# indianajohn/akaze-rust

Hardware: AMD Instinct MI355X
Metric: Mpix/s through extract_features (4 oct x 4 sub) (higher is better)
Workload: dtype f32

## Files before the change

akaze-rust_amd/csrc/akz_ctx.hpp:

```cpp
#pragma once
#include <algorithm>
#include <cmath>
#include <cstdlib>
#include <cstddef>
#include <cstring>
#include <atomic>
#include <condition_variable>
#include <functional>
#include <map>
#include <memory>
#include <mutex>
#include <thread>
#include <sched.h>
#include <time.h>
#include <type_traits>

#include "akz_internal.hpp"
#include "akz_select.hpp"
#include "akz_pool.hpp"
#include "akz_gates.hpp"

#define AKZ_LOCAL __attribute__((visibility("hidden")))

namespace akz {
// ... 51 lines not shown
    DevBuf kp_in, kp_out;
    DevBuf match_a, match_b, match_rec, match_out;
    DevBuf match_state;
    uint32_t match_epoch = 0;
    DevBuf ransac_dev, ransac_pin;
    DevBuf mm_q8, mm_t8, mm_pop, mm_tab;
    DevBuf mm_cols;
    void* tab_ring = nullptr;
    size_t tab_ring_bytes = 0;
    uint64_t tab_ring_next = 0;
    hipEvent_t tab_ring_ev[4] = {nullptr, nullptr, nullptr, nullptr};
    struct MatchSide {
        DevBuf q8, t8, pop, tab, cols, rec;
        void* ring = nullptr;
        size_t ring_bytes = 0;
        uint64_t ring_next = 0;
        hipEvent_t ring_ev[4] = {nullptr, nullptr, nullptr, nullptr};
    } ms1;
    int match_mode = 2;
    uint32_t dbg_pair_chunks = 0, dbg_set_chunks = 0;
    int dbg_device_libm = -1;
    int libm_last = 0;
    int dbg_host_sort = -1;
    DevBuf cosi;
    DevBuf pin[10];
    std::vector<std::pair<size_t, void*>> slab_pool;
    std::mutex slab_m;
    static constexpr int kSlots = 3;
    DevBuf cand_slot[kSlots], count_slot[kSlots];
    std::atomic<bool> slot_busy[kSlots] = {{false}, {false}, {false}};
    std::atomic<uint32_t> cand_cap_hint{1u << 15};
    std::atomic<int> live_results{0};
    bool dead = false;
    std::atomic<uint32_t> last_total_cands{0};
    std::atomic<uint64_t> last_cand_shape{0};
    hipStream_t aux = nullptr;
    std::mutex aux_m;
    hipStream_t coarse = nullptr;
    hipStream_t pre = nullptr;
    hipEvent_t pre_done = nullptr;
    hipStream_t copy = nullptr;
    DevBuf stage[kSlots];
    hipEvent_t staged[kSlots] = {nullptr, nullptr, nullptr};
    std::vector<akz_ctx*> lanes;
    unsigned next_lane = 0;
    bool is_lane = false;
    bool eager_finish = true;
    std::shared_ptr<Finisher> fin;
    hipEvent_t lane_in = nullptr;
    uint64_t stream_min_px = gates::kStreamPx;
    int prep_mode = 2;
    int det_mode = 2;
    int fed_mode = 2;
    int sched[11] = {0, 1, 0, 0, 0, 0, 0, 0, 0, 0, 0};
    uint64_t big_px = gates::kBigPxAsync;
    uint64_t big_px_sync = gates::kBigPxSync, big_px_async = gates::kBigPxAsync;
    uint64_t lane_px = gates::kLanePx;
    static constexpr uint64_t kLaunchMarchPx = gates::kMarchPx;
    uint64_t launch_min_px = kLaunchMarchPx;
    bool placed = false;
    int pre_mode = 0;
    int place_replaced = 0;
    int place_collisions = 0;
    int place_retries = 0;
    int lane_collisions = 0;
    hipEvent_t probe_ev[2] = {nullptr, nullptr};
    int profiling = 0;
    akz_profile prof{};
    struct Span { int stage; hipEvent_t a, b; int row; };
    std::vector<Span> spans;
    std::vector<akz_kernel_row> rows;
    std::vector<hipEvent_t> ev_pool;
    std::mutex ev_m;
    static constexpr int kFedRing = 4;
    hipEvent_t fed_ev[kFedRing] = {nullptr, nullptr, nullptr, nullptr};
    hipEvent_t pre_ev[kFedRing] = {nullptr, nullptr, nullptr, nullptr};
    std::atomic<uint64_t> begin_seq{0};
    std::shared_ptr<std::atomic<int>> in_hand = std::make_shared<std::atomic<int>>(0);
    std::unique_ptr<WorkerPool> workers;
    unsigned host_threads = 0;
    WorkerPool& pool() {
        if (!workers) workers.reset(new WorkerPool(std::min(host_threads ? host_threads : host_cpu_share(), 16u) - 1));
        return *workers;
    }
    hipStream_t fetch[2] = {nullptr, nullptr};
    DevBuf fetch_stage;
    hipEvent_t fetch_chunk[4] = {nullptr, nullptr, nullptr, nullptr};
    DevBuf fetch_tmp[3], fetch_out[2][4];
    hipEvent_t fetch_start = nullptr, fetch_join = nullptr, fetch_ready[2] = {nullptr, nullptr}, fetch_free[2] = {nullptr, nullptr};
    static constexpr int kJpegSlots = 16;
    DevBuf jpeg_pin[kJpegSlots];
    hipEvent_t jpeg_up[kJpegSlots] = {};
    DevBuf jpeg_coef, jpeg_plane, jpeg_frames;
    std::mutex jpeg_m;
};
constexpr int kStageIngest = 10;

struct StageTimer {
    akz_ctx* c;
    int stage;
    hipEvent_t a = nullptr, b = nullptr;
    static hipEvent_t get(akz_ctx* c) {
        {
            std::lock_guard<std::mutex> lk(c->ev_m);
            if (!c->ev_pool.empty()) {
                hipEvent_t e = c->ev_pool.back();
                c->ev_pool.pop_back();
// ... 169 lines not shown
```

akaze-rust_amd/csrc/akz_extract.cpp:

```cpp
#include "akz_ctx.hpp"

struct akz_result {
    akz_ctx* ctx = nullptr;
    akz_config cfg;
    uint32_t w = 0, h = 0, n = 0, flags = 0;
    uint64_t big_px = 0;
    std::vector<LevelPlan> plan;
    void* slab = nullptr;
    size_t slab_bytes = 0;
    float* planes[kMaxLevels][10];
    double* d_k = nullptr;
    std::vector<double> k_host;
    std::vector<std::vector<akz_keypoint>> kps;
    std::vector<uint8_t> rows64;
    uint8_t* d_desc64 = nullptr;
    size_t desc_block_bytes = 0;
    std::vector<uint64_t> desc_off;
    std::vector<uint64_t> n_extrema;
};

static size_t align_up(size_t v, size_t a) { return (v + a - 1) / a * a; }

static int slab_acquire(akz_ctx* c, size_t bytes, void** p, size_t* got) {
    bytes = align_up(std::max<size_t>(bytes, 256), 256);
// ... 498 lines not shown
    std::vector<char> prepared(L + 1, 0);
    const uint64_t level_min_px = gates::kLevelMarchPx;
    auto takes_level_march = [&](size_t l) {
        return !plan[l].tau.empty() && c->fed_mode == 2 && launch::level_march_supported(plan[l].w, plan[l].h) &&
               (c->prep_mode == 3 || (c->prep_mode == 2 && (uint64_t)plan[l].w * plan[l].h * n >= level_min_px));
    };
    auto takes_stream_prep = [&](size_t l) {
        const bool half_l = plan[l].octave > plan[l - 1].octave;
        return c->prep_mode != 0 && launch::prep_stream_supported(plan[l].w, plan[l].h) &&
               (c->prep_mode == 1 || (c->prep_mode >= 2 && !half_l && (uint64_t)plan[l].w * plan[l].h * n >= c->stream_min_px));
    };
    auto run_levels = [&](size_t lo, size_t hi) -> int {
    for (size_t i = lo; i < hi; ++i) {
        const LevelPlan& lv = plan[i];
        const LevelPlan& pv = plan[i - 1];
        if (i >= 2) interleave_detector(i - 1);

        if (i == res_first) {
            std::vector<launch::ResidentLevel> rl;
            std::vector<std::vector<float>> ht(L);
            uint64_t px_steps = 0;
            for (size_t l = i; l < L; ++l) {
                for (double t : plan[l].tau) ht[l].push_back(0.5f * (float)t);
                rl.push_back(launch::ResidentLevel{P(l, AKZ_LT), P(l, AKZ_LSMOOTH), P(l, AKZ_LFLOW), keep_all ? P(l, AKZ_LSTEP) : nullptr,
                                                   plan[l].w, plan[l].h, plan[l].octave > plan[l - 1].octave,
                                                   (uint32_t)plan[l].tau.size(), ht[l].data(), plan[l].octave});
                px_steps += (uint64_t)plan[l].w * plan[l].h * n * plan[l].tau.size();
            }
            StageTimer st(c, AKZ_ST_FED);
            st.kernel(AKZ_KR_OCTAVE_RESIDENT, (uint32_t)rl.size(), plan[i].w, plan[i].h, n, 1, 0, px_steps);
            launch::octave_resident(ls, P(i - 1, AKZ_LT), pv.w, pv.h, n, rl.data(), (uint32_t)rl.size(), g1.data(), r->d_k);
            if (c->profiling) {
                c->prof.fed_launches += 1;
                c->prof.fed_px_steps += px_steps;
            }
            AKZ_HIP_TRY(hipGetLastError());
            break;
        }
        float* A = P(i, AKZ_LT);
        const bool on_coarse = i >= fork_level;
        if (on_coarse) AKZ_TRY(ensure(c, c->scratch_coarse, plane_bytes(plan[fork_level].w, plan[fork_level].h, n)));
        float* B = (float*)(on_coarse ? c->scratch_coarse.p : c->scratch[5].p);
        const uint32_t n_tau = (uint32_t)lv.tau.size();
        const bool half = lv.octave > pv.octave;
        const float* fed_in = P(i - 1, AKZ_LT);
        float* half_buf = nullptr;
        if (half) {
            const uint32_t launches = fed_num_launches(c, n_tau, lv.w, lv.h, n);
            half_buf = launches == 0 ? A : (fed_dst(launches, 1, A, B) == A ? B : A);
            fed_in = half_buf;
        }
        const bool fuse_level = takes_level_march(i);
        if (fuse_level) {
            const uint32_t n1 = std::min<uint32_t>(n_tau, 4u), rem = n_tau - n1;
            const uint32_t rest = rem ? fed_num_launches(c, rem, lv.w, lv.h, n) : 0;
            float* d1 = fed_dst(rest + 1, 1, A, B);
            const float* level_in = P(i - 1, AKZ_LT);
            const bool fold_half = half && launch::level_march_half_supported(lv.w, lv.h, pv.w, pv.h, n1);
            if (half && !fold_half) {
                StageTimer st(c, AKZ_ST_PREP);
                float* hb = d1 == A ? B : A;
                launch::half_size(ls, P(i - 1, AKZ_LT), hb, pv.w, pv.h, n);
                level_in = hb;
            }
            float ht[4];
            for (uint32_t j = 0; j < n1; ++j) ht[j] = 0.5f * (float)lv.tau[j];
            {
                StageTimer st(c, AKZ_ST_FED);
                st.kernel(AKZ_KR_LEVEL_MARCH, n1 | (fold_half ? 16u : 0u) | ((rem == 0 && keep_all) ? 32u : 0u), lv.w, lv.h, n, 1,
                          (uint64_t)lv.w * lv.h * n, (uint64_t)lv.w * lv.h * n * n1);
                launch::level_march(ls, level_in, P(i, AKZ_LSMOOTH), P(i, AKZ_LFLOW), d1,
                                    (rem == 0 && keep_all) ? P(i, AKZ_LSTEP) : nullptr, lv.w, lv.h, n, g1.data(), r->d_k,
                                    lv.octave, ht, n1, fold_half ? pv.w : 0u, fold_half ? pv.h : 0u);
                if (c->profiling) {
                    c->prof.fed_launches += 1;
                    c->prof.fed_px_steps += (uint64_t)lv.w * lv.h * n * n1;
                    c->prof.fused_px += (uint64_t)lv.w * lv.h * n;
                }
            }
            if (rem) {
                StageTimer st(c, AKZ_ST_FED);
                st.kernel(AKZ_KR_FED_OWN, rem, lv.w, lv.h, n, rest, 0, (uint64_t)lv.w * lv.h * n * rem);
                AKZ_TRY(fed_impl(c, d1, A, B, P(i, AKZ_LFLOW), keep_all ? P(i, AKZ_LSTEP) : nullptr, lv.w, lv.h, n,
                                 lv.tau.data() + n1, rem));
            }
            AKZ_HIP_TRY(hipGetLastError());
            continue;
        }
        if (i == 1 && head_level1) {
            StageTimer st(c, AKZ_ST_PREP);
            launch::flow_from_pair(ls, P(0, AKZ_LX), P(0, AKZ_LY), P(1, AKZ_LFLOW), lv.w, lv.h, n, r->d_k, lv.octave);
        } else if (!prepared[i]) {
            StageTimer st(c, AKZ_ST_PREP);
            const bool stream_prep = takes_stream_prep(i);
            if (stream_prep)
                launch::prep_stream(ls, P(i - 1, AKZ_LT), half, half_buf, P(i, AKZ_LSMOOTH), P(i, AKZ_LFLOW), lv.w, lv.h,
                                    pv.w, pv.h, n, g1.data(), r->d_k, lv.octave);
            else
                launch::prep_fused(ls, P(i - 1, AKZ_LT), half, half_buf, P(i, AKZ_LSMOOTH), P(i, AKZ_LFLOW), lv.w, lv.h,
                                   pv.w, pv.h, n, g1.data(), r->d_k, lv.octave);
        }
        if (keep_all && n_tau == 0) AKZ_HIP_TRY(hipMemsetAsync(P(i, AKZ_LSTEP), 0, plane_bytes(lv.w, lv.h, n), ls));
        {
            launch::FedNextPrep np{};
            const bool ride = c->sched[6] == 0 && c->fed_mode == 2 && i + 1 < L && i + 1 != res_first && plan[i + 1].octave == lv.octave &&
                              !takes_level_march(i + 1) && !takes_stream_prep(i + 1);
            if (ride) np = launch::FedNextPrep{P(i + 1, AKZ_LSMOOTH), P(i + 1, AKZ_LFLOW), g1.data(), r->d_k, plan[i + 1].octave};
            bool rode = false;
            StageTimer st(c, AKZ_ST_FED);
            st.kernel(AKZ_KR_FED_OWN, n_tau, lv.w, lv.h, n, fed_num_launches(c, n_tau, lv.w, lv.h, n), 0, (uint64_t)lv.w * lv.h * n * n_tau);
            AKZ_TRY(fed_impl(c, fed_in, A, B, P(i, AKZ_LFLOW), keep_all ? P(i, AKZ_LSTEP) : nullptr, lv.w, lv.h, n,
                             lv.tau.data(), n_tau, ride ? &np : nullptr, &rode));
            prepared[i + 1] = rode ? 1 : 0;
        }
    }
    return AKZ_OK;
    };

// ... 1560 lines not shown
```

akaze-rust_amd/csrc/akz_internal.hpp:

```cpp
#pragma once
#include <hip/hip_runtime.h>

#include <cstdint>
#include <functional>
#include <string>
#include <vector>

#include "../../include/akaze_hip.h"
#include "../../include/akaze_hip_debug.h"

namespace akz {

void set_error(const std::string& msg);
unsigned host_cpu_share();

using TrialsOnDevice = std::function<int(const float*, const float*, const float*, const float*, uint32_t, const uint32_t*, uint32_t,
                                         float, float, float*, int32_t*)>;
int remove_outliers_impl(const akz_keypoint* keypoints_0, uint64_t n0, const akz_keypoint* keypoints_1, uint64_t n1,
                         const akz_match* matches, uint64_t n_matches, uint64_t num_trials, float epsilon_model,
                         float epsilon_inlier, akz_match* out, uint64_t* n_out, const TrialsOnDevice& trials_on_device);

#define AKZ_HIP_TRY(expr)                                                                          \
    do {                                                                                           \
        hipError_t _e = (expr);                                                                    \
// ... 126 lines not shown
                    uint32_t ntaps);
void blur_fused_u8(hipStream_t s, const uint8_t* in, float* out, uint32_t w, uint32_t h, uint32_t n, const float* k,
                   uint32_t ntaps);
void prep_fused(hipStream_t s, const float* prev, bool half, float* lt_out, float* lsmooth, float* lflow, uint32_t w,
                uint32_t h, uint32_t pw, uint32_t ph, uint32_t n, const float* g3, const double* d_k, uint32_t k_pow);
bool detector_fused_supported(uint32_t sigma);
void detector_fused(hipStream_t s, const float* lsmooth, uint32_t sigma, float* lx, float* ly, float* lxx, float* lyy,
                    float* lxy, float* ldet_out, uint32_t w, uint32_t h, uint32_t n);
bool detector_tiled_fused_supported(uint32_t sigma);
struct DetLevelDesc {
    const float* lsmooth;
    float *lx, *ly, *lxx, *lyy, *lxy, *ldet;
    uint32_t w, h, level;
    float border_m;
};
uint32_t detector_tiled_set_max();
void detector_tiled_set(hipStream_t s, uint32_t sigma, const DetLevelDesc* levels, uint32_t nlevels, uint32_t n, float thr,
                        Candidate* d_cand, uint32_t cap, uint32_t* d_count);
void detector_tiled_fused(hipStream_t s, const float* lsmooth, uint32_t sigma, float* lx, float* ly, float* lxx,
                          float* lyy, float* lxy, float* ldet_out, uint32_t w, uint32_t h, uint32_t n, uint32_t level,
                          float thr, float border_m, Candidate* d_cand, uint32_t cap, uint32_t* d_count);
bool blur5_stream_supported(uint32_t w, uint32_t h, uint32_t ntaps, bool is_u8);
void blur5_stream_u8(hipStream_t s, const uint8_t* in, float* out, uint32_t w, uint32_t h, uint32_t n, const float* k);
void blur5_stream_f32(hipStream_t s, const float* in, float* out, uint32_t w, uint32_t h, uint32_t n, const float* k);
uint32_t march_band_rows(int kind, uint32_t w, uint32_t h, uint32_t n, int S, int32_t* cs_ce, uint32_t cap);
bool blur5_march_supported(uint32_t w, uint32_t h, uint32_t ntaps);
void blur5_march_u8(hipStream_t s, const uint8_t* in, float* out, uint32_t w, uint32_t h, uint32_t n, const float* k);
void blur5_march_f32(hipStream_t s, const float* in, float* out, uint32_t w, uint32_t h, uint32_t n, const float* k);
bool contrast_march_supported(uint32_t w, uint32_t h, uint32_t ntaps, uint32_t nbins);
void contrast_march(hipStream_t s, const float* in, uint32_t w, uint32_t h, uint32_t n, const float* g3,
                    unsigned long long* d_hmax_bits, uint32_t nbins, uint32_t* d_hist, double* d_thr);
void contrast_thresholds(hipStream_t s, const unsigned long long* d_hmax_bits, uint32_t nbins, uint32_t n, double* d_thr);
bool contrast_stream_supported(uint32_t w, uint32_t h, uint32_t ntaps, uint32_t nbins);
void contrast_stream(hipStream_t s, const float* in, uint32_t w, uint32_t h, uint32_t n, const float* g3,
                     unsigned long long* d_hmax_bits, uint32_t nbins, uint32_t* d_hist, double* d_thr);
bool prep_stream_supported(uint32_t w, uint32_t h);
void prep_stream(hipStream_t s, const float* prev, bool half, float* lt_out, float* lsmooth, float* lflow, uint32_t w,
                 uint32_t h, uint32_t pw, uint32_t ph, uint32_t n, const float* g3, const double* d_k, uint32_t k_pow);
bool detector_march_supported(uint32_t sigma, uint32_t w, uint32_t h, float border_m, bool nms);
void detector_march(hipStream_t s, const float* lsmooth, uint32_t sigma, float* lx, float* ly, float* lxx, float* lyy,
                    float* lxy, float* ldet_out, uint32_t w, uint32_t h, uint32_t n, uint32_t level, float thr,
                    float border_m, Candidate* d_cand, uint32_t cap, uint32_t* d_count);
bool head_fused_supported(uint32_t w, uint32_t h, uint32_t ntaps0, uint32_t ntaps1);
void head_fused_u8(hipStream_t s, const uint8_t* in, float* lt0, float* blurred, float* gx, float* gy, uint32_t w, uint32_t h, uint32_t n,
                   const float* k5, const float* g3, unsigned long long* d_smax_bits, uint32_t* d_zero_word = nullptr);
void head_fused_f32(hipStream_t s, const float* in, float* lt0, float* blurred, float* gx, float* gy, uint32_t w, uint32_t h, uint32_t n,
                    const float* k5, const float* g3, unsigned long long* d_smax_bits, uint32_t* d_zero_word = nullptr);
void contrast_hist_final(hipStream_t s, const float* gx, const float* gy, uint32_t w, uint32_t h, uint32_t n, unsigned long long* d_smax_bits,
                         uint32_t nbins, uint32_t* d_hist, uint32_t* d_done, double percentile, double* d_k);
void flow_from_pair(hipStream_t s, const float* gx, const float* gy, float* lflow, uint32_t w, uint32_t h, uint32_t n, const double* d_k,
                    uint32_t k_pow);
void march_min_band_rows(int detector, int level);
bool level_march_supported(uint32_t w, uint32_t h);
bool level_march_half_supported(uint32_t w, uint32_t h, uint32_t pw, uint32_t ph, uint32_t n_steps);
void level_march(hipStream_t s, const float* prev, float* lsmooth, float* lflow, float* lt_out, float* lstep, uint32_t w,
                 uint32_t h, uint32_t n, const float* g3, const double* d_k, uint32_t k_pow, const float* half_taus,
                 uint32_t n_steps, uint32_t pw = 0, uint32_t ph = 0);
struct ResidentLevel {
    float *lt, *lsmooth, *lflow, *lstep;
    uint32_t w, h;
    bool half;
    uint32_t n_tau;
    const float* half_tau;
    uint32_t k_pow;
};
constexpr int kResidentMaxLevels = 10;
constexpr int kResidentMaxSteps = 448;
bool octave_resident_supported(uint32_t w, uint32_t h);
void octave_resident(hipStream_t s, const float* prev, uint32_t pw, uint32_t ph, uint32_t n, const ResidentLevel* levels,
                     uint32_t n_levels, const float* g3, const double* d_k);
bool detector_nms_fused_supported(uint32_t sigma);
void detector_nms_fused(hipStream_t s, const float* lsmooth, uint32_t sigma, float* lx, float* ly, float* lxx,
                        float* lyy, float* lxy, float* ldet_out, uint32_t w, uint32_t h, uint32_t n, uint32_t level,
                        float thr, float border_m, Candidate* d_cand, uint32_t cap, uint32_t* d_count);
void rcp_f64_to_f32(hipStream_t s, const double* x, float* out, uint64_t n);
void accumulate(hipStream_t s, float* a, const float* b, uint64_t count);
void ldet(hipStream_t s, const float* lxx, const float* lyy, const float* lxy, float* out, uint64_t count,
          float sigma_quat);
size_t sort_candidates_scratch(uint32_t cap, uint64_t max_px, uint32_t n_levels, uint32_t n_images);
uint32_t sort_small_capacity();
size_t sort_candidates_buckets_scratch(uint32_t cap);
bool sort_candidates_buckets(hipStream_t s, const Candidate* d_cand, uint32_t cap, const uint32_t* d_count, const uint32_t* level_w,
                             const uint32_t* level_h, uint32_t n_levels, uint32_t n_images, void* scratch, bool scratch_is_new,
                             Candidate* d_sorted, uint32_t* d_zero, void* rel_scratch);
bool sort_candidates_rows(hipStream_t s, const Candidate* d_cand, uint32_t cap, const uint32_t* d_count, const uint32_t* level_w,
                          const uint32_t* level_h, uint32_t n_levels, Candidate* d_sorted, uint32_t* d_zero, void* rel_scratch);
bool sort_candidates_device(hipStream_t s, const Candidate* d_cand, uint32_t cap, const uint32_t* d_count, uint64_t max_px,
                            uint32_t n_levels, uint32_t n_images, void* scratch, Candidate* d_sorted, uint32_t* d_zero = nullptr);
size_t candidate_relations_bytes(uint32_t cap, const uint32_t* level_h, uint32_t n_levels, uint32_t n_images);
void candidate_relations(hipStream_t s, const Candidate* d_sorted, uint32_t cap, const uint32_t* d_count, const float* size, const float* ratio,
                         const uint32_t* level_w, const uint32_t* level_h, uint32_t n_levels, uint32_t n_images, void* scratch,
                         uint16_t** d_rel_out, uint32_t** d_flags_out, void* sel_scratch = nullptr, bool tables_ready = false);
size_t select_device_bytes(uint32_t cap, uint32_t n_images);
uint32_t* select_device_revcnt(void* sel_scratch, uint32_t cap, uint32_t n_images);
void select_device(hipStream_t s, const Candidate* d_sorted, uint32_t cap, const uint32_t* d_count, const float* size, const float* ratio,
                   const uint32_t* level_w, const uint32_t* level_h, uint32_t n_levels, uint32_t n_images, const void* rel_scratch,
                   void* sel_scratch, const double* d_k, void* d_recs, KpParam* d_pars, uint32_t** d_hdr_out, uint32_t** d_total_out);
void nms(hipStream_t s, const float* ldet, uint32_t w, uint32_t h, uint32_t n, uint64_t img_stride, uint32_t level,
         float thr, float border_m, Candidate* d_cand, uint32_t cap, uint32_t* d_count);
void orientation(hipStream_t s, const LevelTable& lt, const KpParam* d_kp, uint32_t nkp,
                 unsigned long long window_mask, uint32_t n_windows, OrientOut* d_out);
void orientation_counted(hipStream_t s, const LevelTable& lt, const KpParam* d_kp, const uint32_t* d_nkp, uint32_t max_kp,
                         unsigned long long window_mask, uint32_t n_windows, OrientOut* d_out, uint32_t out_stride);
void mldb(hipStream_t s, const LevelTable& lt, const KpParam* d_kp, const float* d_cosi, uint32_t nkp,
          uint32_t channels, uint8_t* d_desc64);
struct MldbMirror {
// ... 83 lines not shown
```

akaze-rust_amd/csrc/akz_march.hip:

```cpp
#include <hip/hip_runtime.h>

#include <algorithm>
#include <cstdlib>
#include <type_traits>

#include "akz_internal.hpp"
#include "akz_pm_g2.hpp"

namespace akz {
namespace {

typedef float f2 __attribute__((ext_vector_type(2)));
typedef float f2u __attribute__((ext_vector_type(2), aligned(4)));

constexpr int MT = 256;
constexpr int MW = 2 * MT;
constexpr int HALO = 16;
constexpr int USE = MW - 2 * HALO;
constexpr int PAD = 8;
constexpr int ROW = MW + 2 * PAD;
constexpr int CBUF = 32;
#ifndef AKZ_MARCH_PF
#define AKZ_MARCH_PF 3
#endif
// ... 273 lines not shown
                    Cc = tap_off(xa, xc);
                }
                rA[k] = A; rB[k] = B; rC[k] = Cc;
                if (u1 == S) {
#pragma unroll
                    for (int d = 1; d <= S; ++d) {
                        rA[(k + P - d) % P] = A; rB[(k + P - d) % P] = B; rC[(k + P - d) % P] = Cc;
                    }
                }
                const f2 lxx = tap_off(rA[k0], rA[k]);
                const f2 lyy = tap_main(rB[k0], rB[k1], rB[k], kn, kwn);
                const f2 lxy = tap_main(rC[k0], rC[k1], rC[k], kn, kwn);
                const f2 det = ((lxx * lyy) - (lxy * lxy)) * quat;
                {
                    f2 o[NOUT];
                    o[0] = det;
                    if (KEEP) { o[1] = lxx; o[2] = lyy; o[3] = lxy; }
                    const f2(&oc)[NOUT] = o;
                    store_filled<S, NOUT, ODDW>(out2c, C, w, h, c, c >= cs && c < ce, oc);
                }
                if (NMS) {
                    const int y = c - 1;
                    if (y >= cs && y < ce && y >= nms.ylo && y <= nms.yhi) {
                        const float* dr = buf + 3 * ROW + wi;
                        const float left = dr[-1], right = dr[2];
                        const bool h0 = (dm1.x > nms.thr) & (dm1.x > dm1.y) & (dm1.x > left) & (dm1.x > dm2.x) & (dm1.x > det.x);
                        const bool h1 = (dm1.y > nms.thr) & (dm1.y > right) & (dm1.y > dm1.x) & (dm1.y > dm2.y) & (dm1.y > det.y);
                        const unsigned m = ((h0 ? 1u : 0u) | (h1 ? 2u : 0u)) & xok;
                        cands_push(cbuf, cnum, m, nms, lane, [&](int i) {
                            Candidate cd;
                            cd.level = nms.level;
                            cd.idx = (unsigned)(y * w + C.x0 + i);
                            cd.v = i == 0 ? dm1.x : dm1.y;
                            cd.xp = i == 0 ? dm1.y : right;
                            cd.xm = i == 0 ? left : dm1.x;
                            cd.yp = i == 0 ? det.x : det.y;
                            cd.ym = i == 0 ? dm2.x : dm2.y;
                            cd.img = (unsigned)img;
                            return cd;
                        });
                    }
                    dm2 = dm1;
                    dm1 = det;
                }
                lx_c = lx_n;
                ly_c = ly_n;
            }
        }
    }
    if (NMS) cands_flush(cbuf, cnum, nms, lane);
}

struct LevelTaus {
    float half_tau[4];
};
__device__ __forceinline__ f2 lds2(const float* p) { return f2{p[0], p[1]}; }
__device__ __forceinline__ f2 tap3(f2 a, f2 b, f2 c, float k0, float k1, float k2) {
    const f2 z = {0.0f, 0.0f};
    return ((z + k0 * a) + k1 * b) + k2 * c;
}
__device__ __forceinline__ double octave_contrast(double k, unsigned pow) {
    for (unsigned i = 0; i < pow; ++i) k = k * 0.75;
    return k;
}

typedef unsigned u4m __attribute__((ext_vector_type(4)));
template <int N, bool KEEPSTEP, bool ODDW, bool HALF = false>
__global__ void __launch_bounds__(MT, 3)
k_level_march(const float* __restrict__ prev, float* __restrict__ lsmooth_out, float* __restrict__ lflow_out,
              float* __restrict__ lt_out, float* __restrict__ lstep_out, int w, int h, MarchGrid g, float g0, float g1,
              float g2, float kn, float kwn, const double* __restrict__ d_k, unsigned k_pow, LevelTaus ht, int pw = 0, int ph = 0) {
    static_assert(!(HALF && ODDW), "the 2x2 mean is folded in for even level widths only");
    static_assert(N >= 1 && N <= 4, "fused diffusion steps");
    static_assert(N + 3 <= HALO, "strip halo");
    constexpr int NPL = 3 + N;
#ifndef AKZ_LEVEL_PF
#define AKZ_LEVEL_PF 2
#endif
    constexpr int PF = AKZ_LEVEL_PF;
    static_assert(PF >= 1 && PF <= 3, "prefetch ring");
    __shared__ __attribute__((aligned(16))) float s_row[2][NPL][ROW];
    const int tid = threadIdx.x;
    const int per = g.nbands * g.nstrips;
    const int cell = march_cell();
    if (cell >= g.total) return;
    const int img = __builtin_amdgcn_readfirstlane(cell / per);
    const int rem = cell - img * per;
    const int band = __builtin_amdgcn_readfirstlane(rem / g.nstrips), strip = rem - band * g.nstrips;
    int cs, ce;
    level_band_rows(g, band, h, &cs, &ce);
    if (cs >= ce) return;
    const int lt0 = cs == 1 ? 0 : cs, lt1 = ce == h - 1 ? h : ce;

    const int X0 = strip * USE - HALO;
    const int p0 = (2 * tid + HALO) & (MW - 1);
    const bool inner = p0 >= HALO && p0 < MW - HALO;
    const Cols C = make_cols(X0 + p0, inner, w);
    const int i0 = PAD + clampi(clampi(C.x0, 1, w - 2) - X0, 0, MW - 1) - 1;
    const int i1 = PAD + clampi(clampi(C.x0 + 1, 1, w - 2) - X0, 0, MW - 1) - 1;
    const int wi = PAD + p0;
    const bool edge_h = __ballot(i0 != wi - 1 || i1 != wi) != 0ull;
    const bool hxn0 = C.x0 > 0, hxp0 = C.x0 + 1 < w, hxn1 = C.x0 + 1 > 0, hxp1 = C.x0 + 2 < w;
    const bool edge_col = __ballot(!(hxn0 && hxp0 && hxn1 && hxp1)) != 0ull;

    const size_t base = (size_t)img * (size_t)w * (size_t)h;
    const __amdgpu_buffer_rsrc_t in = HALF ? plane_rsrc(prev + (size_t)img * (size_t)pw * (size_t)ph, pw, ph) : plane_rsrc(prev + base, w, h);
    const __amdgpu_buffer_rsrc_t o_ls[1] = {plane_rsrc(lsmooth_out + base, w, h)};
    const __amdgpu_buffer_rsrc_t o_lf[1] = {plane_rsrc(lflow_out + base, w, h)};
    __amdgpu_buffer_rsrc_t o_lt[KEEPSTEP ? 2 : 1];
    o_lt[0] = plane_rsrc(lt_out + base, w, h);
    if (KEEPSTEP) o_lt[1] = plane_rsrc(lstep_out + base, w, h);
    const __amdgpu_buffer_rsrc_t(&o_ltc)[KEEPSTEP ? 2 : 1] = o_lt;
    const double kc = octave_contrast(d_k[img], k_pow);
    const double inverse_k = 1.0 / (kc * kc);

    const int v0 = lt0 - N - 2;
    const int T = (lt1 - lt0) + 2 * N + 6;
    struct Fed {
        f2 v;
        u4m top, bot;
    };
    auto feed = [&](int t) -> Fed {
        Fed f;
        const unsigned row = (unsigned)clampi(v0 + min(t, T - 1), 0, h - 1);
        if constexpr (HALF) {
            const unsigned ro = 2u * row * ((unsigned)pw * 4u);
            f.top = __builtin_amdgcn_raw_buffer_load_b128(in, (int)(2u * C.vo_ld), (int)ro, 0);
            f.bot = __builtin_amdgcn_raw_buffer_load_b128(in, (int)(2u * C.vo_ld), (int)(ro + (unsigned)pw * 4u), 0);
        } else {
            f.v = load_pair<ODDW>(in, row * ((unsigned)w * 4u), C);
        }
        return f;
    };
    auto pair_of = [&](const Fed& f) -> f2 {
        if constexpr (HALF) {
            float a = 0.0f, b = 0.0f;
            a = a + __uint_as_float(f.top.x); a = a + __uint_as_float(f.bot.x); a = a + __uint_as_float(f.top.y); a = a + __uint_as_float(f.bot.y);
            b = b + __uint_as_float(f.top.z); b = b + __uint_as_float(f.bot.z); b = b + __uint_as_float(f.top.w); b = b + __uint_as_float(f.bot.w);
            return f2{a / 4.0f, b / 4.0f};
        } else {
            return f.v;
        }
    };
    Fed q[4];
#pragma unroll
    for (int i = 0; i < PF; ++i) q[i] = feed(i);
    const f2 zero = {0.0f, 0.0f};
    f2 LP[8], CR[8];
    f2 GH[4], HM[4], HO[4];
    f2 SXW[4], SXE[4];
    f2 W[N > 1 ? N - 1 : 1][4];
#pragma unroll
    for (int i = 0; i < 8; ++i) LP[i] = CR[i] = zero;
#pragma unroll
    for (int i = 0; i < 4; ++i) {
        GH[i] = HM[i] = HO[i] = SXW[i] = SXE[i] = zero;
#pragma unroll
        for (int j = 0; j < (N > 1 ? N - 1 : 1); ++j) W[j][i] = zero;
    }
    f2 ls_c = zero, lf_c = zero, gh_c = zero;

    auto rows = [&](auto mid_tag) {
    constexpr bool MID = decltype(mid_tag)::value;
    for (int t0 = 0; t0 < T; t0 += 8) {
#pragma unroll
        for (int k = 0; k < 8; ++k) {
            const int t = t0 + k;
            {
                const int v = v0 + t;
                q[(k + PF) & 3] = feed(t + PF);
                float* const buf = &s_row[t & 1][0][0];
                LP[k & 7] = fix_pair(pair_of(q[k & 3]), C);
                *reinterpret_cast<f2*>(buf + 0 * ROW + wi) = LP[k & 7];
                *reinterpret_cast<f2*>(buf + 1 * ROW + wi) = ls_c;
                *reinterpret_cast<f2*>(buf + 2 * ROW + wi) = CR[(k - 5) & 7];
                *reinterpret_cast<f2*>(buf + 3 * ROW + wi) = LP[(k - 5) & 7];
#pragma unroll
                for (int s = 2; s <= N; ++s) *reinterpret_cast<f2*>(buf + (2 + s) * ROW + wi) = W[s - 2][(k - 1) & 3];
                __syncthreads();
                f2 gh = gh_c;
                if (MID || v <= h - 2) {
                    f2 a, b, c;
                    if (!rare(edge_h)) {
                        a = lds2(buf + wi - 1); b = LP[k & 7]; c = lds2(buf + wi + 1);
                    } else {
                        const float* r0 = buf + i0;
                        const float* r1 = buf + i1;
                        a = f2{r0[0], r1[0]}; b = f2{r0[1], r1[1]}; c = f2{r0[2], r1[2]};
                    }
                    gh = tap3(a, b, c, g0, g1, g2);
                }
                gh_c = gh;
                GH[k & 3] = gh;
                if (!MID && rare(v == 1)) GH[(k - 1) & 3] = gh;
                const int u = v - 1;
                f2 ls_n = ls_c;
                if (MID || u <= h - 2) ls_n = tap3(GH[(k - 2) & 3], GH[(k - 1) & 3], GH[k & 3], g0, g1, g2);
                {
                    const f2 o[1] = {ls_n};
                    if (MID) store_rows<1, ODDW>(o_ls, u, w, u >= cs && u < ce, C, o);
                    else store_filled<1, 1, ODDW>(o_ls, C, w, h, u, u >= cs && u < ce, o);
                }
                {
                    f2 a, b, c;
                    if (!rare(edge_h)) {
                        a = lds2(buf + ROW + wi - 1); b = ls_c; c = lds2(buf + ROW + wi + 1);
                    } else {
                        const float* r0 = buf + ROW + i0;
                        const float* r1 = buf + ROW + i1;
                        a = f2{r0[0], r1[0]}; b = f2{r0[1], r1[1]}; c = f2{r0[2], r1[2]};
                    }
                    HM[k & 3] = tap_main(a, b, c, kn, kwn);
                    HO[k & 3] = tap_off(a, c);
                }
                if (!MID && rare(u - 1 == 1)) {
                    HM[(k - 1) & 3] = HM[k & 3];
                    HO[(k - 1) & 3] = HO[k & 3];
                }
                const int c = v - 3;
                f2 lf_n = lf_c;
                if (MID || c <= h - 2) {
                    const f2 lx1 = tap_off(HM[(k - 2) & 3], HM[k & 3]);
                    const f2 ly1 = tap_main(HO[(k - 2) & 3], HO[(k - 1) & 3], HO[k & 3], kn, kwn);
                    lf_n = f2{pm_g2_px(lx1.x, ly1.x, inverse_k), pm_g2_px(lx1.y, ly1.y, inverse_k)};
                }
                CR[(k - 3) & 7] = lf_n;
                if (!MID && rare(c == 1)) CR[(k - 4) & 7] = lf_n;
                {
                    const f2 o[1] = {lf_n};
                    if (MID) store_rows<1, ODDW>(o_lf, c, w, c >= cs && c < ce, C, o);
                    else store_filled<1, 1, ODDW>(o_lf, C, w, h, c, c >= cs && c < ce, o);
                }
                {
                    const float* cr = buf + 2 * ROW + wi;
                    const f2 cc = CR[(k - 5) & 7];
                    SXW[k & 3] = lds2(cr - 1) + cc;
                    SXE[k & 3] = cc + lds2(cr + 1);
                }
                f2 lnew = zero, st = zero;
#pragma unroll
                for (int s = 1; s <= N; ++s) {
                    const int r = v - 4 - s;
                    f2 Lm, Lc, Lp;
                    if (s == 1) {
                        Lm = LP[(k - 6) & 7]; Lc = LP[(k - 5) & 7]; Lp = LP[(k - 4) & 7];
                    } else {
                        W[s - 2][k & 3] = lnew;
                        Lm = W[s - 2][(k - 2) & 3]; Lc = W[s - 2][(k - 1) & 3]; Lp = lnew;
                    }
                    const float* lr = buf + (2 + s) * ROW + wi;
                    const f2 Lw = lds2(lr - 1), Le = lds2(lr + 1);
                    const f2 cN = CR[(k - 5 - s) & 7], cC = CR[(k - 4 - s) & 7], cS = CR[(k - 3 - s) & 7];
                    const f2 SU = cN + cC, SV = cC + cS;
                    const f2 XFW = SXW[(k - (s - 1)) & 3] * (Lc - Lw);
                    const f2 XFE = SXE[(k - (s - 1)) & 3] * (Le - Lc);
                    f2 tx;
                    if (!edge_col) {
                        tx = XFE - XFW;
                    } else {
                        tx.x = hxp0 ? (hxn0 ? XFE.x - XFW.x : XFE.x) : -XFW.x;
                        tx.y = hxp1 ? (hxn1 ? XFE.y - XFW.y : XFE.y) : -XFW.y;
                    }
                    f2 tt;
                    if (MID || r + 1 < h) {
                        tt = tx + SV * (Lp - Lc);
                        if (MID || r > 0) tt = tt - SU * (Lc - Lm);
                    } else {
                        tt = tx + SU * (Lm - Lc);
                    }
                    st = ht.half_tau[s - 1] * tt;
                    lnew = Lc + st;
                }
                {
                    const int r = v - 4 - N;
                    {
                        f2 o[KEEPSTEP ? 2 : 1];
                        o[0] = lnew;
                        if constexpr (KEEPSTEP) o[1] = st;
                        const f2(&oc)[KEEPSTEP ? 2 : 1] = o;
                        store_rows<KEEPSTEP ? 2 : 1, ODDW>(o_ltc, r, w, r >= lt0 && r < lt1, C, oc);
                    }
                }
                ls_c = ls_n;
                lf_c = lf_n;
            }
        }
    }
    };
    const int v_last = v0 + ((T + 7) & ~7) - 1;
    if (v0 >= N + 5 && v_last <= h - 2) rows(std::true_type{});
    else rows(std::false_type{});
}

struct ContrastMarchArgs {
    unsigned long long* hmax_bits;
    unsigned* hist;
    unsigned nbins;
    const double* thr;
};
constexpr int CM_COPIES = 2;
template <int MODE, bool ODDW>
__global__ void __launch_bounds__(MT, 8)
k_contrast_march(const float* __restrict__ in_plane, int w, int h, MarchGrid g, float g0, float g1, float g2, float kn,
                 float kwn, ContrastMarchArgs ca) {
    constexpr int PF = 2;
    __shared__ __attribute__((aligned(16))) float s_row[2][2][ROW];
    extern __shared__ __attribute__((aligned(16))) unsigned s_chist[];
    const int tid = threadIdx.x, lane = tid & 63, wv = tid >> 6;
// ... 402 lines not shown
    blur5_march_t<uint8_t>(s, in, out, w, h, n, k);
}
void blur5_march_f32(hipStream_t s, const float* in, float* out, uint32_t w, uint32_t h, uint32_t n, const float* k) {
    blur5_march_t<float>(s, in, out, w, h, n, k);
}

bool contrast_march_supported(uint32_t w, uint32_t h, uint32_t ntaps, uint32_t nbins) {
    return ntaps == 3 && nbins >= 1 && nbins <= 640 && level_march_supported(w, h);
}
void contrast_march(hipStream_t s, const float* in, uint32_t w, uint32_t h, uint32_t n, const float* g3,
                    unsigned long long* d_hmax_bits, uint32_t nbins, uint32_t* d_hist, double* d_thr) {
    const Taps m = taps_scharr_main(1);
    const ContrastMarchArgs ca{d_hmax_bits, d_hist, nbins, d_thr};
    dim3 gr;
    const MarchGrid mg = plan_level_march(w, h, n, &gr, 8, g_head_min_rows > 0 ? g_head_min_rows : 32);
    if (w & 1u)
        hipLaunchKernelGGL((k_contrast_march<1, true>), gr, dim3(MT), 0, s, in, (int)w, (int)h, mg, g3[0], g3[1], g3[2], m.wgt[0], m.wgt[1], ca);
    else
        hipLaunchKernelGGL((k_contrast_march<1, false>), gr, dim3(MT), 0, s, in, (int)w, (int)h, mg, g3[0], g3[1], g3[2], m.wgt[0], m.wgt[1], ca);
    contrast_thresholds(s, d_hmax_bits, nbins, n, d_thr);
    const size_t lds = ((size_t)(MT / 64) * CM_COPIES * nbins) * sizeof(unsigned) + (size_t)(nbins + 1) * sizeof(double);
    if (w & 1u)
        hipLaunchKernelGGL((k_contrast_march<2, true>), gr, dim3(MT), lds, s, in, (int)w, (int)h, mg, g3[0], g3[1], g3[2], m.wgt[0], m.wgt[1], ca);
    else
        hipLaunchKernelGGL((k_contrast_march<2, false>), gr, dim3(MT), lds, s, in, (int)w, (int)h, mg, g3[0], g3[1], g3[2], m.wgt[0], m.wgt[1], ca);
}

#ifndef AKZ_LVL_FILL
#define AKZ_LVL_FILL 3
#endif
static int level_min_band_rows(uint32_t w, uint32_t h, uint32_t n) {
    if (g_lvl_min_rows > 0) return g_lvl_min_rows;
    return (uint64_t)w * h * n < (48u << 20) ? 20 : 64;
}
uint32_t march_band_rows(int kind, uint32_t w, uint32_t h, uint32_t n, int S, int32_t* cs_ce, uint32_t cap) {
    dim3 gr;
    const MarchGrid g = kind == 1 ? plan_level_march(w, h, n, &gr, AKZ_LVL_FILL, level_min_band_rows(w, h, n)) : plan_march(w, h, n, S, &gr);
    for (int b = 0; b < g.nbands && (uint32_t)b < cap; ++b) {
        int cs, ce;
        if (kind == 1) level_band_rows(g, b, (int)h, &cs, &ce);
        else uniform_band_rows(g, b, S, (int)h, &cs, &ce);
        cs_ce[2 * b] = cs;
        cs_ce[2 * b + 1] = ce;
    }
    return (uint32_t)g.nbands;
}

bool level_march_supported(uint32_t w, uint32_t h) { return w >= 16 && h >= 16 && (uint64_t)w * h <= (1ull << 28); }

template <int NS, bool KEEPSTEP>
static void launch_level_march(hipStream_t s, dim3 gr, const MarchGrid& mg, const float* prev, float* lsmooth, float* lflow,
                               float* lt_out, float* lstep, uint32_t w, uint32_t h, const float* g3, const Taps& m,
                               const double* d_k, uint32_t k_pow, const LevelTaus& ht, uint32_t pw, uint32_t ph) {
    if constexpr (NS == 4) {
        if (pw) {
            hipLaunchKernelGGL((k_level_march<NS, KEEPSTEP, false, true>), gr, dim3(MT), 0, s, prev, lsmooth, lflow, lt_out, lstep, (int)w,
                               (int)h, mg, g3[0], g3[1], g3[2], m.wgt[0], m.wgt[1], d_k, k_pow, ht, (int)pw, (int)ph);
            return;
        }
    }
    if (w & 1u)
        hipLaunchKernelGGL((k_level_march<NS, KEEPSTEP, true>), gr, dim3(MT), 0, s, prev, lsmooth, lflow, lt_out, lstep, (int)w,
                           (int)h, mg, g3[0], g3[1], g3[2], m.wgt[0], m.wgt[1], d_k, k_pow, ht);
    else
        hipLaunchKernelGGL((k_level_march<NS, KEEPSTEP, false>), gr, dim3(MT), 0, s, prev, lsmooth, lflow, lt_out, lstep, (int)w,
                           (int)h, mg, g3[0], g3[1], g3[2], m.wgt[0], m.wgt[1], d_k, k_pow, ht);
}
#define AKZ_LEVEL(NS)                                                                                                        \
    case NS: {                                                                                                               \
        if (lstep) launch_level_march<NS, true>(s, gr, mg, prev, lsmooth, lflow, lt_out, lstep, w, h, g3, m, d_k, k_pow, ht, pw, ph);  \
        else launch_level_march<NS, false>(s, gr, mg, prev, lsmooth, lflow, lt_out, lstep, w, h, g3, m, d_k, k_pow, ht, pw, ph);       \
    } break;

bool level_march_half_supported(uint32_t w, uint32_t h, uint32_t pw, uint32_t ph, uint32_t n_steps) {
    return n_steps == 4 && (pw & 3u) == 0 && (w & 1u) == 0 && w == pw / 2 && h == ph / 2 && (uint64_t)pw * ph <= (1ull << 28);
}
void level_march(hipStream_t s, const float* prev, float* lsmooth, float* lflow, float* lt_out, float* lstep, uint32_t w,
                 uint32_t h, uint32_t n, const float* g3, const double* d_k, uint32_t k_pow, const float* half_taus,
                 uint32_t n_steps, uint32_t pw, uint32_t ph) {
    const Taps m = taps_scharr_main(1);
    LevelTaus ht;
    for (uint32_t i = 0; i < 4; ++i) ht.half_tau[i] = i < n_steps ? half_taus[i] : 0.0f;
    dim3 gr;
    const MarchGrid mg = plan_level_march(w, h, n, &gr, AKZ_LVL_FILL, level_min_band_rows(w, h, n));
    switch (n_steps) {
        AKZ_LEVEL(1) AKZ_LEVEL(2) AKZ_LEVEL(3) AKZ_LEVEL(4)
        default: break;
    }
}
#undef AKZ_LEVEL

}
}
```

Before: 14270.

## Extend fused level-march kernel to handle up to eight diffusion steps

Raises the number of FED diffusion steps fused into the level-march kernel from four to eight. Levels with more than four tau steps then need fewer separate FED launches and fewer full-image read/write passes. The register ring buffers (CR, SXW/SXE) grow, and the unroll factor doubles when the step count needs it, which raises register pressure and can lower occupancy. A sched flag restores the old four-step cap.

```diff
diff --git a/akaze-rust_amd/csrc/akz_ctx.hpp b/akaze-rust_amd/csrc/akz_ctx.hpp
--- a/akaze-rust_amd/csrc/akz_ctx.hpp
+++ b/akaze-rust_amd/csrc/akz_ctx.hpp
@@ -127,7 +127,7 @@
     int prep_mode = 2;
     int det_mode = 2;
     int fed_mode = 2;
-    int sched[11] = {0, 1, 0, 0, 0, 0, 0, 0, 0, 0, 0};
+    int sched[12] = {0, 1, 0, 0, 0, 0, 0, 0, 0, 0, 0, 0};
     uint64_t big_px = gates::kBigPxAsync;
     uint64_t big_px_sync = gates::kBigPxSync, big_px_async = gates::kBigPxAsync;
     uint64_t lane_px = gates::kLanePx;
diff --git a/akaze-rust_amd/csrc/akz_extract.cpp b/akaze-rust_amd/csrc/akz_extract.cpp
--- a/akaze-rust_amd/csrc/akz_extract.cpp
+++ b/akaze-rust_amd/csrc/akz_extract.cpp
@@ -574,7 +574,8 @@
         }
         const bool fuse_level = takes_level_march(i);
         if (fuse_level) {
-            const uint32_t n1 = std::min<uint32_t>(n_tau, 4u), rem = n_tau - n1;
+            const uint32_t cap = c->sched[11] == 1 ? 4u : (uint32_t)launch::kLevelMarchMaxSteps;
+            const uint32_t n1 = std::min<uint32_t>(n_tau, cap), rem = n_tau - n1;
             const uint32_t rest = rem ? fed_num_launches(c, rem, lv.w, lv.h, n) : 0;
             float* d1 = fed_dst(rest + 1, 1, A, B);
             const float* level_in = P(i - 1, AKZ_LT);
@@ -585,7 +586,7 @@
                 launch::half_size(ls, P(i - 1, AKZ_LT), hb, pv.w, pv.h, n);
                 level_in = hb;
             }
-            float ht[4];
+            float ht[launch::kLevelMarchMaxSteps];
             for (uint32_t j = 0; j < n1; ++j) ht[j] = 0.5f * (float)lv.tau[j];
             {
                 StageTimer st(c, AKZ_ST_FED);
diff --git a/akaze-rust_amd/csrc/akz_internal.hpp b/akaze-rust_amd/csrc/akz_internal.hpp
--- a/akaze-rust_amd/csrc/akz_internal.hpp
+++ b/akaze-rust_amd/csrc/akz_internal.hpp
@@ -202,6 +202,7 @@
                     uint32_t k_pow);
 void march_min_band_rows(int detector, int level);
 bool level_march_supported(uint32_t w, uint32_t h);
+constexpr int kLevelMarchMaxSteps = 8;
 bool level_march_half_supported(uint32_t w, uint32_t h, uint32_t pw, uint32_t ph, uint32_t n_steps);
 void level_march(hipStream_t s, const float* prev, float* lsmooth, float* lflow, float* lt_out, float* lstep, uint32_t w,
                  uint32_t h, uint32_t n, const float* g3, const double* d_k, uint32_t k_pow, const float* half_taus,
diff --git a/akaze-rust_amd/csrc/akz_march.hip b/akaze-rust_amd/csrc/akz_march.hip
--- a/akaze-rust_amd/csrc/akz_march.hip
+++ b/akaze-rust_amd/csrc/akz_march.hip
@@ -349,7 +349,7 @@
 }
 
 struct LevelTaus {
-    float half_tau[4];
+    float half_tau[8];
 };
 __device__ __forceinline__ f2 lds2(const float* p) { return f2{p[0], p[1]}; }
 __device__ __forceinline__ f2 tap3(f2 a, f2 b, f2 c, float k0, float k1, float k2) {
@@ -368,7 +368,7 @@
               float* __restrict__ lt_out, float* __restrict__ lstep_out, int w, int h, MarchGrid g, float g0, float g1,
               float g2, float kn, float kwn, const double* __restrict__ d_k, unsigned k_pow, LevelTaus ht, int pw = 0, int ph = 0) {
     static_assert(!(HALF && ODDW), "the 2x2 mean is folded in for even level widths only");
-    static_assert(N >= 1 && N <= 4, "fused diffusion steps");
+    static_assert(N >= 1 && N <= 8, "fused diffusion steps");
     static_assert(N + 3 <= HALO, "strip halo");
     constexpr int NPL = 3 + N;
 #ifndef AKZ_LEVEL_PF
@@ -439,19 +439,26 @@
             return f.v;
         }
     };
+    constexpr int NC = N + 3 <= 8 ? 8 : 16;
+    constexpr int NX = N <= 4 ? 4 : 8;
+    constexpr int U = NC;
     Fed q[4];
 #pragma unroll
     for (int i = 0; i < PF; ++i) q[i] = feed(i);
     const f2 zero = {0.0f, 0.0f};
-    f2 LP[8], CR[8];
+    f2 LP[8], CR[NC];
     f2 GH[4], HM[4], HO[4];
-    f2 SXW[4], SXE[4];
+    f2 SXW[NX], SXE[NX];
     f2 W[N > 1 ? N - 1 : 1][4];
 #pragma unroll
-    for (int i = 0; i < 8; ++i) LP[i] = CR[i] = zero;
+    for (int i = 0; i < 8; ++i) LP[i] = zero;
+#pragma unroll
+    for (int i = 0; i < NC; ++i) CR[i] = zero;
+#pragma unroll
+    for (int i = 0; i < NX; ++i) SXW[i] = SXE[i] = zero;
 #pragma unroll
     for (int i = 0; i < 4; ++i) {
-        GH[i] = HM[i] = HO[i] = SXW[i] = SXE[i] = zero;
+        GH[i] = HM[i] = HO[i] = zero;
 #pragma unroll
         for (int j = 0; j < (N > 1 ? N - 1 : 1); ++j) W[j][i] = zero;
     }
@@ -459,10 +466,11 @@
 
     auto rows = [&](auto mid_tag) {
     constexpr bool MID = decltype(mid_tag)::value;
-    for (int t0 = 0; t0 < T; t0 += 8) {
-#pragma unroll
-        for (int k = 0; k < 8; ++k) {
+    for (int t0 = 0; t0 < T; t0 += U) {
+#pragma unroll
+        for (int k = 0; k < U; ++k) {
             const int t = t0 + k;
+            if (k == 8 && t >= T) break;
             {
                 const int v = v0 + t;
                 q[(k + PF) & 3] = feed(t + PF);
@@ -470,7 +478,7 @@
                 LP[k & 7] = fix_pair(pair_of(q[k & 3]), C);
                 *reinterpret_cast<f2*>(buf + 0 * ROW + wi) = LP[k & 7];
                 *reinterpret_cast<f2*>(buf + 1 * ROW + wi) = ls_c;
-                *reinterpret_cast<f2*>(buf + 2 * ROW + wi) = CR[(k - 5) & 7];
+                *reinterpret_cast<f2*>(buf + 2 * ROW + wi) = CR[(k - 5) & (NC - 1)];
                 *reinterpret_cast<f2*>(buf + 3 * ROW + wi) = LP[(k - 5) & 7];
 #pragma unroll
                 for (int s = 2; s <= N; ++s) *reinterpret_cast<f2*>(buf + (2 + s) * ROW + wi) = W[s - 2][(k - 1) & 3];
@@ -521,8 +529,8 @@
                     const f2 ly1 = tap_main(HO[(k - 2) & 3], HO[(k - 1) & 3], HO[k & 3], kn, kwn);
                     lf_n = f2{pm_g2_px(lx1.x, ly1.x, inverse_k), pm_g2_px(lx1.y, ly1.y, inverse_k)};
                 }
-                CR[(k - 3) & 7] = lf_n;
-                if (!MID && rare(c == 1)) CR[(k - 4) & 7] = lf_n;
+                CR[(k - 3) & (NC - 1)] = lf_n;
+                if (!MID && rare(c == 1)) CR[(k - 4) & (NC - 1)] = lf_n;
                 {
                     const f2 o[1] = {lf_n};
                     if (MID) store_rows<1, ODDW>(o_lf, c, w, c >= cs && c < ce, C, o);
@@ -530,9 +538,9 @@
                 }
                 {
                     const float* cr = buf + 2 * ROW + wi;
-                    const f2 cc = CR[(k - 5) & 7];
-                    SXW[k & 3] = lds2(cr - 1) + cc;
-                    SXE[k & 3] = cc + lds2(cr + 1);
+                    const f2 cc = CR[(k - 5) & (NC - 1)];
+                    SXW[k & (NX - 1)] = lds2(cr - 1) + cc;
+                    SXE[k & (NX - 1)] = cc + lds2(cr + 1);
                 }
                 f2 lnew = zero, st = zero;
 #pragma unroll
@@ -547,10 +555,10 @@
                     }
                     const float* lr = buf + (2 + s) * ROW + wi;
                     const f2 Lw = lds2(lr - 1), Le = lds2(lr + 1);
-                    const f2 cN = CR[(k - 5 - s) & 7], cC = CR[(k - 4 - s) & 7], cS = CR[(k - 3 - s) & 7];
+                    const f2 cN = CR[(k - 5 - s) & (NC - 1)], cC = CR[(k - 4 - s) & (NC - 1)], cS = CR[(k - 3 - s) & (NC - 1)];
                     const f2 SU = cN + cC, SV = cC + cS;
-                    const f2 XFW = SXW[(k - (s - 1)) & 3] * (Lc - Lw);
-                    const f2 XFE = SXE[(k - (s - 1)) & 3] * (Le - Lc);
+                    const f2 XFW = SXW[(k - (s - 1)) & (NX - 1)] * (Lc - Lw);
+                    const f2 XFE = SXE[(k - (s - 1)) & (NX - 1)] * (Le - Lc);
                     f2 tx;
                     if (!edge_col) {
                         tx = XFE - XFW;
@@ -1059,7 +1067,7 @@
 static void launch_level_march(hipStream_t s, dim3 gr, const MarchGrid& mg, const float* prev, float* lsmooth, float* lflow,
                                float* lt_out, float* lstep, uint32_t w, uint32_t h, const float* g3, const Taps& m,
                                const double* d_k, uint32_t k_pow, const LevelTaus& ht, uint32_t pw, uint32_t ph) {
-    if constexpr (NS == 4) {
+    if constexpr (NS >= 4) {
         if (pw) {
             hipLaunchKernelGGL((k_level_march<NS, KEEPSTEP, false, true>), gr, dim3(MT), 0, s, prev, lsmooth, lflow, lt_out, lstep, (int)w,
                                (int)h, mg, g3[0], g3[1], g3[2], m.wgt[0], m.wgt[1], d_k, k_pow, ht, (int)pw, (int)ph);
@@ -1080,18 +1088,18 @@
     } break;
 
 bool level_march_half_supported(uint32_t w, uint32_t h, uint32_t pw, uint32_t ph, uint32_t n_steps) {
-    return n_steps == 4 && (pw & 3u) == 0 && (w & 1u) == 0 && w == pw / 2 && h == ph / 2 && (uint64_t)pw * ph <= (1ull << 28);
+    return n_steps >= 4 && n_steps <= (uint32_t)kLevelMarchMaxSteps && (pw & 3u) == 0 && (w & 1u) == 0 && w == pw / 2 && h == ph / 2 && (uint64_t)pw * ph <= (1ull << 28);
 }
 void level_march(hipStream_t s, const float* prev, float* lsmooth, float* lflow, float* lt_out, float* lstep, uint32_t w,
                  uint32_t h, uint32_t n, const float* g3, const double* d_k, uint32_t k_pow, const float* half_taus,
                  uint32_t n_steps, uint32_t pw, uint32_t ph) {
     const Taps m = taps_scharr_main(1);
     LevelTaus ht;
-    for (uint32_t i = 0; i < 4; ++i) ht.half_tau[i] = i < n_steps ? half_taus[i] : 0.0f;
+    for (uint32_t i = 0; i < 8; ++i) ht.half_tau[i] = i < n_steps ? half_taus[i] : 0.0f;
     dim3 gr;
     const MarchGrid mg = plan_level_march(w, h, n, &gr, AKZ_LVL_FILL, level_min_band_rows(w, h, n));
     switch (n_steps) {
-        AKZ_LEVEL(1) AKZ_LEVEL(2) AKZ_LEVEL(3) AKZ_LEVEL(4)
+        AKZ_LEVEL(1) AKZ_LEVEL(2) AKZ_LEVEL(3) AKZ_LEVEL(4) AKZ_LEVEL(5) AKZ_LEVEL(6) AKZ_LEVEL(7) AKZ_LEVEL(8)
         default: break;
     }
 }
```

New measurement: 14050, median of 2. -1.5%, worse.
